# ChenWu98/cycle-diffusion

Measured on AMD Instinct MI355X. Metric: images/sec, SD-v1.4 512px CycleDiffusion 100+100 steps, 1/2/4/8 MI355X, higher is better.
Workload: dtype fp16; 1 GPU; C2: Stable-Diffusion-v1.4-shaped U-Net + KL-f8 VAE, 512x512, custom_steps=99 white_box_steps=100 eta=0.1 skip 0, 1 trial, encoder scale 1, decoder CFG 3; batch_per_gpu=4, global_batch=4, parallelism=dp1, steps_per_launch_set=5, launch_set_cap=16, launch_sets_in_flight_per_gpu=1, images_in_flight_per_gpu=20, distributed=single process, weights=synthetic(seed=0)

## Files before the change

### cycle-diffusion_amd/_ffi.py

```python
import ctypes as C
import os

import numpy as np

_HERE = os.path.dirname(os.path.abspath(__file__))
LIB_PATH = os.path.join(_HERE, "lib", "libcyclediff.so")

CD_NET_UNET_OPENAI, CD_NET_UNET_HO, CD_NET_VAE_KL, CD_NET_CLIP_TEXT, CD_NET_BERT_XTR = 1, 2, 3, 4, 5
CD_NET_OCLIP_TEXT, CD_NET_OCLIP_VISION, CD_NET_INCEPTION_FID, CD_NET_LPIPS = 6, 7, 8, 9
CD_SCHED_DDIM, CD_SCHED_DDPM = 0, 1
CD_PREC_16, CD_PREC_F32, CD_PREC_F32X3 = 0, 1, 2
CD_MASK_QSAMPLE, CD_MASK_ENCODER = 0, 1
MASK_SOURCES = {"q_sample": CD_MASK_QSAMPLE, "encoder": CD_MASK_ENCODER}
ACT_NONE, ACT_SILU, ACT_GELU, ACT_GEGLU, ACT_QGELU, ACT_RELU = 0, 1, 2, 3, 4, 5


class NetDesc(C.Structure):
    _fields_ = [
        ("kind", C.c_int), ("image_size", C.c_int), ("in_channels", C.c_int), ("out_channels", C.c_int),
        ("model_channels", C.c_int), ("num_res_blocks", C.c_int),
        ("n_mult", C.c_int), ("channel_mult", C.c_int * 8),
        ("n_attn", C.c_int), ("attn", C.c_int * 8),
        ("num_heads", C.c_int), ("num_head_channels", C.c_int),
        ("use_spatial_transformer", C.c_int), ("context_dim", C.c_int), ("transformer_depth", C.c_int),
# ... 66 lines not shown
    "cd_net_create": [_VP, C.POINTER(NetDesc), C.POINTER(_I)],
    "cd_net_param_count": [_VP, _I, C.POINTER(_I)],
    "cd_net_param_info": [_VP, _I, _I, C.c_char_p, _I, C.POINTER(_I), C.POINTER(_I64)],
    "cd_net_load_param": [_VP, _I, C.c_char_p, _VP, _I, C.POINTER(_I64)],
    "cd_net_missing_params": [_VP, _I, C.POINTER(_I), C.c_char_p, _I],
    "cd_unet_forward": [_VP, _I, _VP, _VP, _VP, _I, _I, _VP],
    "cd_text_encode": [_VP, _I, _VP, _I, _I, _VP],
    "cd_clip_text_features": [_VP, _I, _VP, _I, _I, _VP],
    "cd_clip_image_features": [_VP, _I, _VP, _I, _VP],
    "cd_inception_features": [_VP, _I, _VP, _I, _I, _VP],
    "cd_lpips": [_VP, _I, _VP, _VP, _I, _I, _I, _VP, _VP],
    "cd_lpips_tap": [_VP, _I, _VP, _I, _I, _I, _I, _VP],
    "cd_vae_encode": [_VP, _I, _VP, _VP, _U64, _I, _I, _I, _F, _VP],
    "cd_vae_decode": [_VP, _I, _VP, _I, _I, _F, _F, _F, _VP],
    "cd_vae_encode_hw": [_VP, _I, _VP, _VP, _U64, _I, _I, _I, _I, _F, _VP],
    "cd_vae_decode_hw": [_VP, _I, _VP, _I, _I, _I, _F, _F, _F, _VP],
    "cd_dpm_encode": [_VP, _I, _I, _VP, _VP, _VP, _I, _F, _I, _I, _VP, _VP, _U64, _I, _VP],
    "cd_ddim_decode": [_VP, _I, _I, _VP, _I, _I, _VP, _VP, _I, _F, _I, _I, _VP, _VP, _U64, _VP],
    "cd_ddim_decode_v": [_VP, _I, _I, _VP, _I, _I, _VP, _VP, _I, _VP, _I, _I, _VP, _VP, _U64, _VP],
    "cd_ddim_invert": [_VP, _I, _I, _VP, _VP, _VP, _I, _F, _I, _I, _VP, _VP, _VP],
    "cd_cycle_translate": [_VP, C.POINTER(TranslateArgs)],
    "cd_ddim_decode_masked": [_VP, _I, _I, _VP, _I, _I, _VP, _VP, _I, _F, _VP, _I, _I, _VP, _VP, _U64, _VP, _VP, _I, _I, _VP, _VP,
                              _U64, _VP],
    "cd_ilvr_decode": [_VP, _I, _I, _VP, _I, _I, _I, _I, _VP, _VP, _U64, _VP, _I, _I, _I, _VP, _VP, _U64, _VP],
    "cd_automask": [_VP, _I, _VP, _VP, _VP, _I, _I, _I, _I, _F, _F, _VP, _U64, _I, _F, _F, _I, _VP, _VP],
    "cd_word_maps": [_VP, _I, _VP, _VP, _I, _I, _VP, _I, _I, _I, _I, _F, _F, _VP, _U64, _I, _I, _I, _VP, C.POINTER(_I)],
    "cd_pix_refine": [_VP, _I, _I, _VP, _I, _I, _VP, _VP, _U64],
    "cd_op_pack_conv_weight": [_VP, _VP, _I, _I, _I, _I, _I, C.POINTER(_VP), C.POINTER(_I), C.POINTER(_I)],
    "cd_op_free": [_VP, _VP],
    "cd_op_conv2d": [_VP, _VP, _I, _VP, _I, _I, _I, _I, _VP, _I, _I, _I, _I, _I, _I, _I, _VP, _VP, _VP, _I, _I, _VP],
    "cd_op_conv2d_16": [_VP, _VP, _I, _VP, _I, _I, _I, _I, _VP, _I, _I, _I, _I, _I, _I, _I, _VP, _VP, _VP, _I, _I, _VP,
                        _VP],
    "cd_op_last_gemm_config": [_VP] + [C.POINTER(_I)] * 5,
    "cd_op_up_phase_reorder": [_VP, _VP, _I, _I, _I, _I, _VP],
    "cd_op_groupnorm": [_VP, _VP, _I, _I, _I, _I, _I, _F, _VP, _VP, _VP, _I, _VP],
    "cd_op_groupnorm_ex": [_VP, _VP, _I, _I, _VP, _I, _I, _I, _I, _I, _F, _VP, _VP, _VP, _I, _I, _VP, _VP, _I, _VP],
    "cd_op_pack_conv_weight_prec": [_VP, _VP, _I, _I, _I, _I, _I, C.POINTER(_VP)],
    "cd_op_conv2d_prec": [_VP, _VP, _I, _I, _VP, _I, _I, _I, _I, _I, _VP, _I, _I, _I, _I, _I, _I, _I, _VP, _VP, _I, _VP, _I, _I,
                          _I, _I, _I, _I, _F, _VP, _VP],
    "cd_op_attention_prec": [_VP, _VP, _VP, _VP, _I, _I, _I, _I, _I, _I, _I, _I, _F, _I, _VP, _I, _I, _VP],
    "cd_op_rows_prec": [_VP, _I, _VP, _I64, _I, _I, _VP, _I, _I, _VP, _VP, _I, _VP],
    "cd_op_resample_prec": [_VP, _I, _VP, _I, _I, _I, _I, _I, _VP],
    "cd_op_layernorm": [_VP, _VP, _I, _I, _VP, _VP, _F, _VP],
    "cd_op_st_entry": [_VP, _VP, _I, _I, _I, _VP, _VP, _F, _VP, _VP, _VP, _VP, _VP, _VP, _VP, _I, _VP, _VP, _VP,
                       C.POINTER(_I)],
    "cd_op_attention": [_VP, _VP, _VP, _VP, _I, _I, _I, _I, _I, _F, _I, _VP],
    "cd_op_cross_attention_ctrl": [_VP, _VP, _VP, _VP, _VP, _VP, _VP, _VP, _VP, _I, _I, _I, _I, _I, _I, _I, _I, _F, _VP],
    "cd_op_cross_attention_ctrl_ex": [_VP, _VP, _VP, _VP, _VP, _VP, _VP, _VP, _VP, _I, _I, _I, _I, _I, _I, _I, _I, _F, _I, _I,
                                      _VP],
    "cd_op_cross_attention_maps": [_VP, _VP, _VP, _VP, _I, _I, _I, _I, _I, _I, _I, _I, _F, _I, _VP],
    "cd_op_attention_ex": [_VP, _VP, _VP, _VP, _I, _I, _I, _I, _I, _I, _I, _I, _I, _I, _F, _I, _VP, _I, _I, _VP],
    "cd_op_lowpass": [_VP, _VP, _I, _I, _I, _I, _VP],
    "cd_op_softmax_rows": [_VP, _VP, _I64, _I, _VP],
    "cd_op_timestep_embedding": [_VP, _VP, _I, _I, _I, _VP],
    "cd_op_sched_step": [_VP, _I, _I, _VP, _VP, _VP, _VP, _I, _F, _VP, _VP, _I, _I, _I, _I, _VP],
    "cd_op_gauss": [_VP, _U64, C.c_uint32, _I64, _I64, _VP],
    "cd_op_automask_reduce": [_VP, _VP, _VP, _I, _I, _I, _I, _I, _F, _F, _I, _VP, _VP, _VP],
    "cd_op_local_blend_mask": [_VP, _VP, _VP, _I, _I, _I, _I, _I, _F, _VP],
    "cd_op_sched_step_masked": [_VP, _I, _VP, _VP, _VP, _I, _F, _VP, _VP, _VP, _I, _I, _F, _F, _VP, _I, _I, _I, _I, _VP, _I],
    "cd_op_sega_guidance": [_VP, _VP, _I, _I, _I, _I, _I, _F, _VP, _VP, _I, _F, _F, _VP, _VP, _VP, _VP, _VP],
    "cd_op_window_gather": [_VP, _VP, _VP, _I, _I, _I, _I, _I, _I, _I, _I, _VP],
    "cd_op_window_fuse": [_VP, _VP, _VP, _I, _I, _I, _I, _I, _I, _I, _I, _VP],
    "cd_op_layout": [_VP, _I, _VP, _VP, _I, _I, _I, _I, _I, _F, _F, _I],
    "cd_op_resample16": [_VP, _I, _VP, _VP, _I, _I, _I, _I],
    "cd_op_copy_rows16": [_VP, _VP, _I, _VP, _I, _I64, _I],
    "cd_op_vec_linear": [_VP, _VP, _I, _VP, _VP, _VP, _I, _I, _I, _I, _I, _I],
# ... 65 lines not shown
```

### cycle-diffusion_amd/csrc/capi_ops.hip

```cpp
#include "capi_internal.h"

namespace {

bf16_t* op_rows16(cd_engine* h, const float* src, int64_t rows, int C) {
  bf16_t* d = (bf16_t*)h->arena.alloc((size_t)rows * C * 2);
  launch_nchw_to_nhwc(h->st, src, d, (int)rows, C, 1, C, 1.f, 0.f, 0);
  return d;
}
Act op_image16(Ctx& c, const float* x, int B, int C, int H, int W, int Cpad) {
  Act a = alloc_act(c, B, H, W, Cpad);
  launch_nchw_to_nhwc(c.st, x, a.p, B, C, H * W, Cpad, 1.f, 0.f, 0);
  return a;
}

bf16_t* op_nan_rows16(cd_engine* h, int64_t rows, int ld) {
  const size_t bytes = (size_t)(rows + 64) * ld * 2;
  bf16_t* t = (bf16_t*)h->arena.alloc(bytes);
  HIP_CHECK(hipMemsetAsync(t, 0xFF, bytes, h->st));
  return t;
}
float* op_nan_buffer(cd_engine* h, size_t n) {
  float* t = (float*)h->arena.alloc(n * sizeof(float));
  launch_fill_f32(h->st, t, __builtin_nanf(""), (int64_t)n);
  return t;
// ... 48 lines not shown
  Act a; a.B = B; a.H = H; a.W = W; a.C = Cpad; a.ld = 2 * Cpad; a.f32 = true; a.split = true;
  a.p = (bf16_t*)h->arena.alloc((size_t)B * H * W * 2 * Cpad * sizeof(bf16_t));
  launch_nchw_to_nhwc_f32(h->st, x, a.pf(), B, C, H * W, Cpad, 1.f, 0.f, 1, h->overflow_dev);
  return a;
}

void op_download_nchw(cd_engine* h, const void* p, bool f32, int ld, float* y, int B, int C, int HW) {
  launch_nhwc_to_nchw(h->st, p, f32 ? 1 : 0, ld, y, B, C, HW, 1.f, 0.f);
}
void op_download(cd_engine* h, const Act& o, size_t floats, void* y) {
  HIP_CHECK(hipMemcpyAsync(y, o.p, floats * 4, hipMemcpyDeviceToDevice, h->st));
  HIP_CHECK(hipStreamSynchronize(h->st));
  h->check_overflow();
}

void conv_out_hw(int H, int W, int KH, int KW, int stride, int pad, bool asym, bool up, int* Ho, int* Wo) {
  const int Hin = up ? 2 * H : H, Win = up ? 2 * W : W;
  *Ho = asym ? (Hin + 1 - KH) / stride + 1 : (Hin + 2 * pad - KH) / stride + 1;
  *Wo = asym ? (Win + 1 - KW) / stride + 1 : (Win + 2 * pad - KW) / stride + 1;
}
Ctx prec_ctx(cd_engine* h, int precision) {
  Ctx c = h->ctx();
  c.f32 = precision != 0; c.x3 = precision == 2;
  return c;
}

void op_conv2d(cd_handle h, const float* x0, int C0, const float* x1, int C1, int B, int H, int W,
               const void* packed_w, int N, int KH, int KW, int stride, int pad, int asym_pad, int up,
               const float* bias, const float* rowvec, const float* resid, int act, int tile, bool out16,
               float* y, float* stats) {
  CD_CHECK(h && x0 && packed_w && y, "bad argument");
  ArenaScope arena_scope(h->arena);
  Ctx c = h->ctx();
  if (up && out16) {
    ConvW* pw = (ConvW*)const_cast<void*>(packed_w);
    h->op_params.add_up_phase(pw);
    h->op_params.refresh_up_phase(h->st, pw);
  }
  ConvW w = *(const ConvW*)packed_w;
  CD_CHECK(w.N == N && w.KH == KH && w.KW == KW, "packed weight does not match the call");
  w.b = const_cast<float*>(bias);
  Act a0 = op_image16(c, x0, B, C0, H, W, x1 ? C0 : round_up(C0, 32));
  Act a1;
  if (x1) a1 = op_image16(c, x1, B, C1, H, W, C1);
  ConvOpts o; o.stride = stride; o.pad = pad; o.asym = asym_pad != 0; o.up = up != 0; o.tile = tile;
  if (act & 0x400) {
    CD_CHECK(out16 && conv_ln_fold_available(c, w, (int64_t)B * H * W) , "LayerNorm fold needs tile 30 shapes");
    o.ln_fold = true;
    act &= ~0x400;
  }
  o.act = act;
  o.out_f32 = !out16;
  o.want_stats = stats != nullptr;
  int Ho, Wo;
  conv_out_hw(H, W, KH, KW, stride, pad, asym_pad != 0, up != 0, &Ho, &Wo);
  const int Nout = w.geglu ? N / 2 : N;
  if (rowvec) { o.rowvec = rowvec; o.rowvec_ld = N; o.rows_per_vec = Ho * Wo; }
  Act r;
  if (resid) {
    r = op_image16(c, resid, B, Nout, Ho, Wo, Nout);
    o.resid = &r;
  }
  Act out = conv_fwd(c, w, a0, x1 ? &a1 : nullptr, o);
  op_download_nchw(h, out.p, !out16, out.ld, y, B, Nout, Ho * Wo);
  if (stats) {
    CD_CHECK(out.stats, "this convolution produces no GroupNorm statistics (GEGLU, or rows %% 32 != 0)");
    HIP_CHECK(hipMemcpyAsync(stats, out.stats, (size_t)(out.rows() / 32) * 2 * Nout * sizeof(float),
                             hipMemcpyDeviceToDevice, h->st));
  }
}

void op_cross_attention_ctrl(cd_engine* h, const float* q_own, const float* q_src, const float* k_own,
                             const float* k_src, const float* v_own, const float* mapper, const float* alpha,
                             const float* weight, int B, int B_src, int B_ctrl, int H, int Tq, int L, int L_buf, int D,
                             float scale, int q_log2, int opad, float* o) {
  CD_CHECK(h && q_own && q_src && k_own && k_src && v_own && mapper && alpha && weight && o, "bad argument");
  CD_CHECK(B > 0 && B_src > 0 && B_ctrl > 0 && H > 0 && Tq > 0 && D > 0 && L > 0 && L_buf >= L, "bad argument");
  CD_CHECK(opad >= 0 && opad % 4 == 0, "opad: a multiple of 4 elements");
  ArenaScope arena_scope(h->arena);
  const int C = H * D, ldo = C + opad;
  CtrlAttnParams p;
  p.q_own = op_rows16(h, q_own, (int64_t)B * Tq, C); p.q_src = op_rows16(h, q_src, (int64_t)B_src * Tq, C);
  p.k_own = op_rows16(h, k_own, (int64_t)B * L_buf, C); p.k_src = op_rows16(h, k_src, (int64_t)B_src * L_buf, C);
  const bf16_t* vb16 = op_rows16(h, v_own, (int64_t)B * L, C);
  bf16_t* va = (bf16_t*)h->arena.alloc((size_t)B * L * C * 2);
  bf16_t* vb = (bf16_t*)h->arena.alloc((size_t)B * L * C * 2);
  launch_ctrl_values(h->st, vb16, mapper, alpha, weight, B, B_ctrl, L, C, va, vb);
  bf16_t* ob = op_nan_rows16(h, (int64_t)B * Tq, ldo);
  p.va = va; p.vb = vb; p.o = ob;
  p.B = B; p.B_src = B_src; p.H = H; p.Tq = Tq; p.L = L; p.D = D;
  p.ldq = C; p.ldk = C; p.ldv = C; p.ldo = ldo;
  p.q_bs = (int64_t)Tq * C; p.k_bs = (int64_t)L_buf * C; p.v_bs = (int64_t)L * C; p.o_bs = (int64_t)Tq * ldo;
  p.scale = scale; p.q_log2 = q_log2 != 0;
  launch_cross_attention_ctrl(h->st, p);
  op_download_nchw(h, ob, false, ldo, o, B * Tq, ldo, 1);
// ... 35 lines not shown
int cd_op_conv2d_16(cd_handle h, const float* x0, int C0, const float* x1, int C1, int B, int H, int W,
                    const void* packed_w, int N, int KH, int KW, int stride, int pad, int asym_pad, int up,
                    const float* bias, const float* rowvec, const float* resid, int act, int tile, float* y,
                    float* stats) {
  CD_API_BEGIN
  enter_engine(h);
  op_conv2d(h, x0, C0, x1, C1, B, H, W, packed_w, N, KH, KW, stride, pad, asym_pad, up, bias, rowvec, resid, act, tile,
            true, y, stats);
  CD_API_END
}

int cd_op_up_phase_reorder(cd_handle h, const float* x, int B, int C, int H, int W, float* y) {
  CD_API_BEGIN
  enter_engine(h);
  CD_CHECK(h && x && y && B > 0 && H > 0 && W > 0 && C > 0 && C % 8 == 0, "bad argument");
  ArenaScope arena_scope(h->arena);
  Ctx c = h->ctx();
  Act a = op_image16(c, x, 4 * B, C, H, W, C);
  Act o = alloc_act(c, B, 2 * H, 2 * W, C);
  launch_up_phase_reorder(h->st, a.p, o.p, B, H, W, C, o.ld);
  op_download_nchw(h, o.p, false, o.ld, y, B, C, 4 * H * W);
  CD_API_END
}

int cd_op_last_gemm_config(cd_handle h, int* tile_id, int* bk, int* splitk, int* chm, int* tile_group) {
  CD_API_BEGIN
  CD_CHECK(h, "bad argument");
  const GemmLaunchInfo li = conv_gemm_last_launch();
  if (tile_id) *tile_id = li.tile_id;
  if (bk) *bk = li.bk;
  if (splitk) *splitk = li.splitk;
  if (chm) *chm = li.chm;
  if (tile_group) *tile_group = li.tile_group;
  CD_API_END
}

int cd_op_groupnorm(cd_handle h, const float* x, int B, int C, int H, int W, int G, float eps,
                    const float* gamma, const float* beta, const float* film, int silu, float* y) {
  CD_API_BEGIN
  enter_engine(h);
  CD_CHECK(h && x && y && G == 32, "bad argument (G must be 32)");
  ArenaScope arena_scope(h->arena);
  Ctx c = h->ctx();
  Act a = op_image16(c, x, B, C, H, W, C);
  GNW w; w.g = const_cast<float*>(gamma); w.b = const_cast<float*>(beta); w.C = C; w.eps = eps;
  Act o = groupnorm_fwd(c, w, a, nullptr, silu != 0, film, film ? 2 * C : 0);
  op_download_nchw(h, o.p, false, o.ld, y, B, C, H * W);
  CD_API_END
}

int cd_op_groupnorm_ex(cd_handle h, const float* x0, int C0, int pad0, const float* x1, int C1, int pad1, int B, int H,
                       int W, float eps, const float* gamma, const float* beta, const float* film, int film_ld, int silu,
                       const float* stats0, const float* stats1, int precision, void* y) {
  CD_API_BEGIN
  enter_engine(h);
  CD_CHECK(h && x0 && gamma && beta && y && B > 0 && H > 0 && W > 0 && C0 > 0 && pad0 >= 0 && pad1 >= 0, "bad argument");
  CD_CHECK(x1 ? C1 > 0 : (C1 == 0 && !stats1), "bad argument (second source)");
  CD_CHECK(precision >= 0 && precision <= 2 && film_ld >= 0, "bad argument (precision 0 = 16-bit, 1 = fp32, 2 = fp32 split)");
  const int align = precision ? 4 : 8;
  CD_CHECK((C0 + pad0) % align == 0 && (C1 + pad1) % align == 0, "row strides must be multiples of %d elements", align);
  ArenaScope arena_scope(h->arena);
  Ctx c = prec_ctx(h, precision);
  const int HW = H * W, C = C0 + C1;
  Act a0 = c.f32 ? op_upload_nhwc(h, x0, B, C0, C0, C0 + pad0, H, W) : op_upload_nhwc16(h, x0, B, C0, C0 + pad0, H, W);
  a0.stats = const_cast<float*>(stats0);
  Act a1;
// ... 942 lines not shown
```

### cycle-diffusion_amd/csrc/conv_gemm.hip

```cpp
#include <stdio.h>
#include <stdlib.h>
#include <string.h>

#include <algorithm>
#include <map>
#include <mutex>
#include <string>

#include "common.h"
#include "kernels.h"

namespace cd {

namespace gemm_detail {

typedef const __attribute__((address_space(1))) void* gptr_t;
typedef __attribute__((address_space(3))) void* lptr_t;

template <int BM, int BN, int BK, int WM, int WN, int NSTAGE>
struct TileCfg {
  static constexpr int NW = WM * WN;
  static constexpr int CPR = BK / 8;
  static constexpr int RPI = 64 / CPR;
  static constexpr int A_IPW = BM / RPI / NW;
  static constexpr int B_IPW = BN / RPI / NW;
  static constexpr int LPT = A_IPW + B_IPW;
  static constexpr int TM = BM / WM, TN = BN / WN;
  static constexpr int MT = TM / 32, NT = TN / 32;
  static constexpr int KS = BK / 16;
  static constexpr int SWZ_SHIFT = (CPR == 8) ? 1 : 2;
  static constexpr int CW = TN >= 64 ? 64 : TN;
  static constexpr int EPI_LD = CW + 4;
  static constexpr int PF = (MT * NT >= 8) ? 1 : 2;
  static constexpr int A_BYTES = BM * BK * 2, B_BYTES = BN * BK * 2;
  static constexpr int STAGE_BYTES = A_BYTES + B_BYTES;
  static constexpr int EPI_BYTES = NW * TM * EPI_LD * 4;
  static constexpr int LDS_BYTES = STAGE_BYTES * NSTAGE > EPI_BYTES ? STAGE_BYTES * NSTAGE : EPI_BYTES;
  static constexpr int TAB_BIAS_I = (BN / 4 + 63) / 64;
  static constexpr int TAB_RV_I = ((BM / 32) * (BN / 4) + 63) / 64;
  static constexpr bool HAS_TAB = LDS_BYTES + (TAB_BIAS_I + TAB_RV_I) * 1024 <= 160 * 1024;
  static constexpr int TAB_BYTES = HAS_TAB ? (TAB_BIAS_I + TAB_RV_I) * 1024 : 0;
  static_assert(NW == 4 || NW == 8 || NW == 16, "4, 8 or 16 waves");
  static_assert(A_IPW >= 1 && B_IPW >= 1, "tile too small for the wave count");
  static_assert(A_IPW * RPI * NW == BM && B_IPW * RPI * NW == BN, "tile rows must split evenly over waves");
  static_assert(MT >= 1 && NT >= 1, "wave tile");
  static_assert(NSTAGE >= 2 && NSTAGE <= 8, "ring depth");
  static_assert((NSTAGE - 2) * LPT <= 63, "vmcnt field");
  static_assert(LDS_BYTES + TAB_BYTES <= 160 * 1024, "LDS");
};

template <int N>
__device__ __forceinline__ void wait_vmcnt_barrier() {
  asm volatile("s_waitcnt vmcnt(%0)\n\ts_barrier" ::"n"(N) : "memory");
}

__device__ __forceinline__ __amdgpu_buffer_rsrc_t uniform_rsrc(const void* base, int bytes) {
  const uint64_t u = (uint64_t)base;
  const uint32_t lo = (uint32_t)__builtin_amdgcn_readfirstlane((int)(uint32_t)u);
  const uint32_t hi = (uint32_t)__builtin_amdgcn_readfirstlane((int)(uint32_t)(u >> 32));
  return __builtin_amdgcn_make_buffer_rsrc((void*)(((uint64_t)hi << 32) | lo), 0, __builtin_amdgcn_readfirstlane(bytes), 0x00020000);
}

__device__ __forceinline__ bool fast_epilogue(const ConvGemmParams& p) {
  return p.act == ACT_NONE && !p.out_f32 && !p.resid_f32 && (p.N & 7) == 0 && (p.out_ld & 7) == 0 &&
         (((uintptr_t)p.out | (uintptr_t)p.resid | (uintptr_t)p.rowvec) & 15) == 0 && (p.o_bs & 7) == 0 &&
         (!p.resid || (p.resid_ld & 7) == 0) &&
         (!p.rowvec || ((p.rowvec_ld & 3) == 0 && (p.rows_per_vec >= p.M || (p.rows_per_vec & 31) == 0)));
}

template <int BM, int BN, int BK, int WM, int WN, int NSTAGE, bool CHM = false>
__global__ __launch_bounds__(64 * WM * WN, (WM * WN == 4 && BK == 32 && NSTAGE == 3 && BM * BN >= 128 * 256) ? 2 : 1) void k_conv_gemm(ConvGemmParams p) {
#if defined(__HIP_DEVICE_COMPILE__)
  using T = TileCfg<BM, BN, BK, WM, WN, NSTAGE>;
  constexpr int CPR = T::CPR, RPI = T::RPI, A_IPW = T::A_IPW, B_IPW = T::B_IPW, NW = T::NW;
  constexpr int MT = T::MT, NT = T::NT, KS = T::KS, TM = T::TM, TN = T::TN, LPT = T::LPT;
  extern __shared__ __attribute__((aligned(16))) char smem[];

  const int tid = threadIdx.x;
  const int lane = tid & 63;
  const int wave = __builtin_amdgcn_readfirstlane(tid >> 6);
  const int wm = wave / WN, wn = wave % WN;

  const int tiles_n = (p.N + BN - 1) / BN;
  const int tiles_m = (p.M + BM - 1) / BM;
  const int ntiles = tiles_m * tiles_n;
  int tile;
  {
    const int bid = blockIdx.x;
    const int q = ntiles >> 3, r = ntiles & 7;
    const int xcd = bid & 7, loc = bid >> 3;
    tile = (xcd < r ? xcd * (q + 1) : r * (q + 1) + (xcd - r) * q) + loc;
  }
  const bool nmajor = (int64_t)p.N * p.Ktot > (int64_t)p.B * p.Hs * p.Ws * (p.C0 + p.C1);
  int tm, tn;
  if (p.tile_group > 0) {
    const int width = p.tile_group * tiles_n;
    const int grp = tile / width, within = tile - grp * width;
    const int first_m = grp * p.tile_group;
    const int gsz = (tiles_m - first_m) < p.tile_group ? (tiles_m - first_m) : p.tile_group;
    tn = within / gsz; tm = first_m + (within - tn * gsz);
  } else if (nmajor) { tn = tile / tiles_m; tm = tile - tn * tiles_m; }
  else { tm = tile / tiles_n; tn = tile - tm * tiles_n; }
  const int m0 = tm * BM, n0 = tn * BN;
// ... 212 lines not shown
  wait_vmcnt_barrier<(NSTAGE - 1) * LPT + TABI>();

  bf16x8 af[KS][MT], bfr[KS][NT];
  auto read_frags = [&](int slot, int ks) {
    const char* Ab = As + slot * T::A_BYTES;
    const char* Bb = Bs + slot * T::B_BYTES;
#pragma unroll
    for (int i = 0; i < MT; ++i) {
      const int row = wm * TM + i * 32 + frow;
      const int ch = (ks * 2 + fhalf) ^ ((row >> T::SWZ_SHIFT) & (CPR - 1));
      af[ks][i] = *(const bf16x8*)(Ab + row * (BK * 2) + ch * 16);
    }
#pragma unroll
    for (int j = 0; j < NT; ++j) {
      const int row = wn * TN + j * 32 + frow;
      const int ch = (ks * 2 + fhalf) ^ ((row >> T::SWZ_SHIFT) & (CPR - 1));
      bfr[ks][j] = *(const bf16x8*)(Bb + row * (BK * 2) + ch * 16);
    }
  };
#pragma unroll
  for (int q = 0; q < PF; ++q) read_frags(0, q);
  __builtin_amdgcn_sched_barrier(0);

  int cur = 0;
  int fill = 0;
  for (int kt = kt0; kt < kt1; ++kt) {
    const int nslot = (cur + 1 == NSTAGE) ? 0 : cur + 1;
#pragma unroll
    for (int ks = 0; ks < KS; ++ks) {
      const int jrel = (ks - SYNC + KS) % KS;
      auto mfma_range = [&](int lo, int hi) __attribute__((always_inline)) {
#pragma unroll
        for (int n = 0; n < NMF; ++n)
          if (n >= lo && n < hi) acc[n / NT][n % NT] = CD_MFMA_32x32x16(af[ks][n / NT], bfr[ks][n % NT], acc[n / NT][n % NT]);
      };
      if (ks == SYNC) {
        mfma_range(0, HALF);
        asm volatile("s_waitcnt vmcnt(%0) lgkmcnt(0)\n\ts_barrier" ::"n"((NSTAGE - 2) * LPT) : "memory");
        prepare(kt + NSTAGE);
        fill = cur;
#pragma unroll
        for (int l = 0; l < LPT / SPREAD; ++l) issue(l, fill);
        mfma_range(HALF, NMF);
      } else {
        if (SPREAD > 1 && (ks > SYNC || kt != kt0)) {
#pragma unroll
          for (int l = (jrel * LPT) / SPREAD; l < ((jrel + 1) * LPT) / SPREAD; ++l) issue(l, fill);
        }
        mfma_range(0, NMF);
      }
      if (ks + PF < KS) read_frags(cur, ks + PF);
      else read_frags(nslot, ks + PF - KS);
      __builtin_amdgcn_sched_barrier(0);
    }
    cur = nslot;
  }
  asm volatile("s_waitcnt vmcnt(0)" ::: "memory");
  __syncthreads();

  if (nsplit > 1) {
    constexpr int TILE_BYTES = BM * BN * 4;
    constexpr int kSc1 = 16;
    typedef __attribute__((ext_vector_type(4))) unsigned int u32x4;
    float* part0 = p.sk_scratch + ((int64_t)zb * ntiles + tile) * nsplit * (BM * BN);
    const __amdgpu_buffer_rsrc_t rsp = __builtin_amdgcn_make_buffer_rsrc((void*)part0, 0, kRange, 0x00020000);
#pragma unroll
    for (int i = 0; i < MT; ++i)
#pragma unroll
      for (int j = 0; j < NT; ++j)
#pragma unroll
        for (int q = 0; q < 4; ++q) {
          const f32x4 v = {acc[i][j][4 * q], acc[i][j][4 * q + 1], acc[i][j][4 * q + 2], acc[i][j][4 * q + 3]};
          const int off = sidx * TILE_BYTES + (((i * NT + j) * 4 + q) * (64 * NW) + tid) * 16;
          __builtin_amdgcn_raw_buffer_store_b128(__builtin_bit_cast(u32x4, v), rsp, off, 0, kSc1);
        }
    asm volatile("s_waitcnt vmcnt(0)" ::: "memory");
    __syncthreads();
    int* flag = p.sk_flags + zb * ntiles + tile;
    if (tid == 0) *(volatile int*)smem = __hip_atomic_fetch_add(flag, 1, __ATOMIC_RELAXED, __HIP_MEMORY_SCOPE_AGENT);
    __syncthreads();
    const int arrived = *(volatile int*)smem;
    __syncthreads();
    if (arrived != nsplit - 1) return;
    if (tid == 0) __hip_atomic_store(flag, 0, __ATOMIC_RELAXED, __HIP_MEMORY_SCOPE_AGENT);
#pragma unroll
    for (int i = 0; i < MT; ++i)
#pragma unroll
      for (int j = 0; j < NT; ++j)
#pragma unroll
        for (int r = 0; r < 16; ++r) acc[i][j][r] = 0.0f;
// ... 346 lines not shown
        }
        if (p.stats) {
#pragma unroll
          for (int e = 0; e < 8; ++e) { ssum[e] += v[e]; ssq[e] += v[e] * v[e]; }
        }
        }
        if (p.stats && ((r0 + rpp) & 31) == 0) {
          for (int o = vpr; o < 64; o <<= 1) {
#pragma unroll
            for (int e = 0; e < 8; ++e) { ssum[e] += __shfl_xor(ssum[e], o); ssq[e] += __shfl_xor(ssq[e], o); }
          }
          const int rb = (m0 + wm * TM + r0 + rpp - 32) >> 5;
          if (vr == 0 && n < p.N && (rb << 5) < p.M) {
            float* sp = p.stats + ((int64_t)zb * ((p.M + 31) >> 5) + rb) * 2 * p.N + n;
#pragma unroll
            for (int e = 0; e < 8; ++e) if (e < nvalid) { sp[e] = ssum[e]; sp[p.N + e] = ssq[e]; }
          }
#pragma unroll
          for (int e = 0; e < 8; ++e) { ssum[e] = 0.f; ssq[e] = 0.f; }
        }
      }
    }
  }
#endif
}


inline bool takes_channel_major(const ConvGemmParams& p) {
  const int64_t a_bytes = (int64_t)p.B * p.Hs * p.Ws * (p.C0 + p.C1) * 2;
  return p.korder != 0 && p.KH * p.KW > 1 && p.KH <= 8 && p.KW <= 8 && !p.up && !p.up_phase &&
         (p.korder == 2 || (p.Hs * p.Ws >= 4096 && a_bytes >= (32ll << 20)));
}

template <int BM, int BN, int BK, int WM, int WN, int NSTAGE>
int launch_cfg(hipStream_t st, const ConvGemmParams& p) {
  using T = TileCfg<BM, BN, BK, WM, WN, NSTAGE>;
  const int tiles = ceil_div(p.M, BM) * ceil_div(p.N, BN);
  const int split = p.splitk > 1 ? p.splitk : 1;
  constexpr int kLds = T::LDS_BYTES + T::TAB_BYTES;
  const bool chm = takes_channel_major(p);
  static PerDeviceOnce attr_once;
  auto kern0 = k_conv_gemm<BM, BN, BK, WM, WN, NSTAGE, false>;
  auto kern1 = k_conv_gemm<BM, BN, BK, WM, WN, NSTAGE, true>;
  attr_once([&]() {
    HIP_CHECK(hipFuncSetAttribute((const void*)kern0, hipFuncAttributeMaxDynamicSharedMemorySize, kLds));
    HIP_CHECK(hipFuncSetAttribute((const void*)kern1, hipFuncAttributeMaxDynamicSharedMemorySize, kLds));
  });
  auto kern = chm ? kern1 : kern0;
  if (split > 1) {
    const SplitKWorkspace& ws = g_conv_splitk;
    CD_CHECK(p.sk_scratch && p.sk_flags, "conv_gemm: split-K without workspace");
    CD_CHECK((size_t)tiles * p.nbatch * split * BM * BN * 4 <= ws.scratch_bytes && tiles * p.nbatch <= ws.nflags,
             "conv_gemm: split-K workspace too small");
  }
  hipLaunchKernelGGL(kern, dim3(tiles, split, p.nbatch), dim3(64 * T::NW), kLds, st, p);
  return 0;
}

struct CfgInfo { int id, BM, BN, TN; const char* name; };
const CfgInfo kCfgs[] = {
    {1, 128, 128, 64, "128x128 w2x2 s2"},
    {2, 128, 64, 64, "128x64 w4x1 s2"},
    {3, 64, 64, 32, "64x64 w2x2 s2"},
    {4, 128, 128, 64, "128x128 w2x2 s3"},
    {5, 256, 128, 64, "256x128 w4x2 s3"},
    {6, 128, 256, 64, "128x256 w2x4 s3"},
    {7, 128, 64, 64, "128x64 w4x1 s4"},
    {8, 64, 64, 32, "64x64 w2x2 s4"},
    {9, 256, 64, 64, "256x64 w8x1 s4"},
    {10, 128, 128, 64, "128x128 w2x2 s4"},
    {11, 64, 128, 64, "64x128 w2x2 s4"},
    {12, 128, 64, 64, "128x64 w4x1 s3"},
    {13, 256, 64, 64, "256x64 w8x1 s3"},
    {14, 128, 128, 64, "128x128 w4x2 s3"},
    {15, 64, 64, 32, "64x64 w2x2 s8"},
    {16, 128, 64, 64, "128x64 w4x1 s6"},
    {17, 64, 128, 64, "64x128 w2x2 s6"},
    {18, 256, 128, 32, "256x128 w4x4 s3"},
    {19, 256, 128, 64, "256x128 w8x2 s3"},
    {20, 256, 320, 160, "256x320 w4x2 s2"},
    {21, 128, 320, 160, "128x320 w2x2 s2"},
// ... 66 lines not shown
thread_local const char* g_last_cfg = "";
thread_local GemmLaunchInfo g_last_launch;

int device_cu_count() {
  static std::atomic<int> ncu_of[64];
  int dev = 0;
  if (hipGetDevice(&dev) != hipSuccess) return 256;
  int n = ncu_of[dev & 63].load(std::memory_order_relaxed);
  if (!n) {
    hipDeviceProp_t prop;
    n = (hipGetDeviceProperties(&prop, dev) == hipSuccess && prop.multiProcessorCount > 0) ? prop.multiProcessorCount : 256;
    ncu_of[dev & 63].store(n, std::memory_order_relaxed);
  }
  return n;
}

int pick_config(const ConvGemmParams& p) {
  const int64_t ncu = device_cu_count();
  const int64_t t128 = (int64_t)ceil_div(p.M, 128) * ceil_div(p.N, 128) * p.nbatch;
  const int64_t t12864 = (int64_t)ceil_div(p.M, 128) * ceil_div(p.N, 64) * p.nbatch;
  if (p.act == ACT_GEGLU) return (2 * t128 >= 3 * ncu) ? 1 : 2;
  if (2 * t128 >= 3 * ncu && p.N % 128 == 0) return 1;
  if (t128 >= 2 * ncu) return 1;
  if (t12864 >= ncu) return 2;
  return 3;
}

}
using namespace gemm_detail;

const char* conv_gemm_last_config() { return g_last_cfg; }
GemmLaunchInfo conv_gemm_last_launch() { return g_last_launch; }

thread_local KernelProfiler* g_conv_prof = nullptr;

void KernelProfiler::next_pair(hipEvent_t* a, hipEvent_t* b, double fl, const std::string& what) {
  labels.push_back(what);
  if (used + 2 > (int)events.size()) {
    const size_t old = events.size();
    events.resize(old + 1024);
    for (size_t i = old; i < events.size(); ++i) HIP_CHECK(hipEventCreate(&events[i]));
  }
  *a = events[used]; *b = events[used + 1];
  used += 2;
  flops.push_back(fl);
}
void KernelProfiler::collect(int* launches, double* total_ms, double* total_flops) {
  double ms = 0, fl = 0;
  for (int i = 0; i + 1 < used; i += 2) {
    HIP_CHECK(hipEventSynchronize(events[i + 1]));
    float t = 0;
    HIP_CHECK(hipEventElapsedTime(&t, events[i], events[i + 1]));
    ms += t; fl += flops[i / 2];
    if (verbose) {
      auto& e = per_shape[labels[i / 2]];
      e.n += 1; e.ms += t; e.flops += flops[i / 2];
    }
  }
  if (verbose) {
    std::vector<std::pair<std::string, Entry>> v(per_shape.begin(), per_shape.end());
    std::sort(v.begin(), v.end(), [](const auto& x, const auto& y) { return x.second.ms > y.second.ms; });
    fprintf(stderr, "[conv_gemm] %d launches %.3f ms %.1f TFLOP/s\n", used / 2, ms, fl / ms * 1e-9);
    for (auto& kv : v)
      fprintf(stderr, "  %-58s n=%4d %8.3f ms %7.1f us/launch %7.1f TF/s\n", kv.first.c_str(), kv.second.n,
              kv.second.ms, kv.second.ms / kv.second.n * 1e3, kv.second.flops / kv.second.ms * 1e-9);
    per_shape.clear();
// ... 276 lines not shown
```

### cycle-diffusion_amd/csrc/kernels.h

```cpp
#pragma once
#include <map>
#include <string>
#include <vector>

#include "common.h"

namespace cd {

struct StepCoef {
  float sa, s1a, sap, dirc, sigma, r, t_mask;
  int t;
};
enum { SCHED_DDIM = 0, SCHED_DDPM = 1 };

struct EpsHat {
  const float* p = nullptr;
  int64_t sb = 0, sc = 0, sp = 0;
  int cfg = 0;
  float g = 1.f;
  const float* gvec = nullptr;
};

struct StepGeom {
  int B = 0, C = 0, HW = 0;
// ... 199 lines not shown
  int act = ACT_NONE;
  void* out = nullptr;
  int out_ld = 0;
  int out_f32 = 0;
  float* stats = nullptr;
  const bf16_t* zeros = nullptr;
  int ln_fold = 0;
  float ln_eps = 1e-5f;
  int tile = 0;
  float prof_flop_scale = 1.f;
  int splitk = 0;
  float* sk_scratch = nullptr;
  int* sk_flags = nullptr;
  int korder = 1;
  int tile_group = 0;
  int up_phase = 0;
  int w_ps = 0;
};
struct SplitKWorkspace {
  float* scratch = nullptr;
  size_t scratch_bytes = 0;
  int* flags = nullptr;
  int nflags = 0;
};
extern thread_local SplitKWorkspace g_conv_splitk;
void launch_conv_gemm(hipStream_t st, const ConvGemmParams& p);
const char* conv_gemm_last_config();
struct GemmLaunchInfo {
  int tile_id = 0;
  int bk = 0;
  int splitk = 1;
  int chm = 0;
  int tile_group = 0;
};
GemmLaunchInfo conv_gemm_last_launch();
void launch_up_phase_weights(hipStream_t st, const bf16_t* w, bf16_t* out, int Npad, int Cpad);
int conv_gemm_num_configs();
const char* conv_gemm_config_name(int id);

struct LinStreamParams {
  const bf16_t* a = nullptr; int lda = 0;
  const bf16_t* wfrag = nullptr;
  const float* bias = nullptr;
  const bf16_t* resid = nullptr; int ldr = 0;
  bf16_t* out = nullptr; int ldo = 0;
  float* stats = nullptr;
  int M = 0, N = 0;
  float ln_eps = 1e-5f;
  int nsplit = 0, hw = 0;
  bf16_t* vt = nullptr; int vt_ld = 0;
  int64_t vt_bytes = 0;
  const float* gn_coef = nullptr;
};
constexpr int kLinStreamTile = 30;
bool lin_stream_supports(const ConvGemmParams& p);
void launch_lin_stream(hipStream_t st, const ConvGemmParams& p);
bool lin_stream_entry_supports(int64_t M, int hw, int lda);
void launch_lin_stream_qkv(hipStream_t st, const bf16_t* a, int lda, int M, int hw, const bf16_t* wfrag, const float* bias,
                           bf16_t* qk, bf16_t* vt, int vt_ld, bool ln_fold, float ln_eps);
void launch_lin_stream_gn(hipStream_t st, const bf16_t* a, int lda, int M, int hw, const float* gn_coef, const bf16_t* wfrag,
                          const float* bias, bf16_t* out, int ldo);
void launch_fold_ln(hipStream_t st, const bf16_t* w, int ldw, const float* gamma, const float* beta, const float* bias,
                    bf16_t* w_out, float* bias_out, int N, int Kc);
void launch_pack_wfrag(hipStream_t st, const bf16_t* w, int ldw, bf16_t* out, int N);

struct KernelProfiler {
  bool enabled = false;
  std::vector<hipEvent_t> events;
// ... 169 lines not shown
```

### include/cyclediff.h

```cpp
#ifndef CYCLEDIFF_H
#define CYCLEDIFF_H
#include <stddef.h>
#include <stdint.h>

#ifdef __cplusplus
extern "C" {
#endif

typedef struct cd_engine* cd_handle;

enum { CD_NET_UNET_OPENAI = 1, CD_NET_UNET_HO = 2, CD_NET_VAE_KL = 3, CD_NET_CLIP_TEXT = 4, CD_NET_BERT_XTR = 5,
       CD_NET_OCLIP_TEXT = 6, CD_NET_OCLIP_VISION = 7, CD_NET_INCEPTION_FID = 8, CD_NET_LPIPS = 9 };
enum { CD_SCHED_DDIM = 0, CD_SCHED_DDPM = 1 };
enum { CD_PREC_16 = 0, CD_PREC_F32 = 1, CD_PREC_F32X3 = 2 };
enum { CD_MASK_QSAMPLE = 0, CD_MASK_ENCODER = 1 };

typedef struct cd_net_desc {
  int kind;
  int image_size;
  int in_channels, out_channels;
  int model_channels;
  int num_res_blocks;
  int n_mult;  int channel_mult[8];
  int n_attn;  int attn[8];
// ... 156 lines not shown
  int n_win;
  const int32_t* win_host;
} cd_translate_args;

int cd_cycle_translate(cd_handle h, const cd_translate_args* a);

int cd_ilvr_decode(cd_handle h, int net, int sched_kind, const float* z, int z_slots, int n_eps, int B, int K,
                   const cd_step_coef* coef_host, const float* noise_tail, uint64_t seed, const float* ref, int B_ref,
                   int down_n, int range_t, const float* qsample_coef_host, const float* ref_noise, uint64_t ref_seed,
                   float* x_out);

int cd_automask(cd_handle h, int net, const float* x0, const float* ctx_src, const float* ctx_tgt, int ctx_len, int B,
                int n_draws, int t, float qa, float qb, const float* noise, uint64_t seed, int max_rows, float ratio, float thr,
                int dilate, float* map_out, float* keep_out);

int cd_word_maps(cd_handle h, int net, const float* x0, const float* ctx, int ctx_len, int B, const float* sel, int B_sel,
                 int N, int n_draws, int t, float qa, float qb, const float* noise, uint64_t seed, int max_rows,
                 int min_side, int max_side, float* maps_out , int* n_layers_out);

int cd_pix_refine(cd_handle h, int net, int sched_kind, float* x, int B, int R,
                  const cd_step_coef* coef_host, const float* noise, uint64_t seed);

int cd_op_pack_conv_weight(cd_handle h, const float* w_host, int N, int Cin, int KH, int KW, int geglu,
                           void** packed_dev, int* Npad, int* Cpad);
int cd_op_free(cd_handle h, void* dev);
int cd_op_conv2d(cd_handle h, const float* x0, int C0, const float* x1, int C1, int B, int H, int W,
                 const void* packed_w, int N, int KH, int KW, int stride, int pad, int asym_pad, int up,
                 const float* bias, const float* rowvec, const float* resid, int act, int tile, float* y);
int cd_op_conv2d_16(cd_handle h, const float* x0, int C0, const float* x1, int C1, int B, int H, int W,
                    const void* packed_w, int N, int KH, int KW, int stride, int pad, int asym_pad, int up,
                    const float* bias, const float* rowvec, const float* resid, int act, int tile, float* y,
                    float* stats);
int cd_op_last_gemm_config(cd_handle h, int* tile_id, int* bk, int* splitk, int* chm, int* tile_group);
int cd_op_up_phase_reorder(cd_handle h, const float* x, int B, int C, int H, int W, float* y);
int cd_op_groupnorm(cd_handle h, const float* x, int B, int C, int H, int W, int G, float eps,
                    const float* gamma, const float* beta, const float* film, int silu, float* y);
int cd_op_groupnorm_ex(cd_handle h, const float* x0, int C0, int pad0, const float* x1, int C1, int pad1, int B, int H,
                       int W, float eps, const float* gamma, const float* beta, const float* film, int film_ld, int silu,
                       const float* stats0, const float* stats1, int precision, void* y);
int cd_op_pack_conv_weight_prec(cd_handle h, const float* w_host, int N, int Cin, int KH, int KW, int geglu,
                                void** packed_dev);
int cd_op_conv2d_prec(cd_handle h, const float* x0, int C0, int pad0, const float* x1, int C1, int pad1, int B, int H, int W,
                      const void* packed_w, int N, int KH, int KW, int stride, int pad, int asym_pad, int up,
                      const float* bias, const float* rowvec, int rowvec_shared, const float* resid, int resid_pad, int act,
                      int raw_geglu, int tile, int precision, int via_split_rows, float alpha, float* y, float* stats);
int cd_op_attention_prec(cd_handle h, const float* q, const float* k, const float* v, int B, int H, int Tq, int Tk, int D,
                         int padq, int padk, int padv, float scale, int q_log2, const float* obias, int mode, int precision,
                         void* o);
int cd_op_rows_prec(cd_handle h, int op, const float* x0, int64_t rows, int C0, int pad0, const float* x1, int C1, int pad1,
                    const float* gamma, const float* beta, int precision, void* y);
int cd_op_resample_prec(cd_handle h, int op, const float* x, int B, int C, int H, int W, int precision, void* y);
int cd_op_layernorm(cd_handle h, const float* x, int rows, int C, const float* gamma, const float* beta,
                    float eps, float* y);
int cd_op_st_entry(cd_handle h, const float* x, int B, int H, int W, const float* gn_gamma, const float* gn_beta,
                   float gn_eps, const void* w_in, const float* b_in, const float* ln_gamma, const float* ln_beta,
                   const void* w_qk, const void* w_v, const float* v_bias, int stages, float* h_out, float* qk_out,
                   float* vt_out, int* stages_run);
int cd_op_attention(cd_handle h, const float* q, const float* k, const float* v, int B, int H, int Tq,
                    int Tk, int D, float scale, int use_transpose_kernel, float* o);
int cd_op_cross_attention_ctrl(cd_handle h, const float* q_own, const float* q_src, const float* k_own, const float* k_src,
                               const float* v_own, const float* mapper, const float* alpha, const float* weight, int B,
                               int B_src, int B_ctrl, int H, int Tq, int L, int L_buf, int D, float scale, float* o);
int cd_op_cross_attention_ctrl_ex(cd_handle h, const float* q_own, const float* q_src, const float* k_own, const float* k_src,
                                  const float* v_own, const float* mapper, const float* alpha, const float* weight, int B,
                                  int B_src, int B_ctrl, int H, int Tq, int L, int L_buf, int D, float scale, int q_log2,
                                  int opad, float* o);
// ... 64 lines not shown
```

Before: 3.591 images/s.

## Add direct-to-global GEGLU epilogue for 256x256x64 conv GEMM tile

Adds a kernel variant for the 256x256 BK64 tile in which the MFMA operands are swapped, so each lane holds rows of output. It then applies the bias from the LDS table and the GEGLU gating in registers, and writes packed bf16 rows straight to global memory with buffer stores and a permlane32 swap. This skips the final __syncthreads and the LDS-staged epilogue for GEGLU feed-forward GEMMs without residual, stats or split-K. The path is on by default, can be switched off through an env var or API call, and adds test hooks for padded output rows. The risk is uncoalesced or partial stores and extra register pressure in the new template instance.

Result: no change. 3.609 images/s, median of 6 (+0.5%).

```diff
diff --git a/cycle-diffusion_amd/_ffi.py b/cycle-diffusion_amd/_ffi.py
--- a/cycle-diffusion_amd/_ffi.py
+++ b/cycle-diffusion_amd/_ffi.py
@@ -122,6 +122,8 @@
     "cd_op_conv2d_16": [_VP, _VP, _I, _VP, _I, _I, _I, _I, _VP, _I, _I, _I, _I, _I, _I, _I, _VP, _VP, _VP, _I, _I, _VP,
                         _VP],
     "cd_op_last_gemm_config": [_VP] + [C.POINTER(_I)] * 5,
+    "cd_op_set_direct_epilogue": [_VP, _I],
+    "cd_op_last_gemm_epilogue": [_VP, C.POINTER(_I)],
     "cd_op_up_phase_reorder": [_VP, _VP, _I, _I, _I, _I, _VP],
     "cd_op_groupnorm": [_VP, _VP, _I, _I, _I, _I, _I, _F, _VP, _VP, _VP, _I, _VP],
     "cd_op_groupnorm_ex": [_VP, _VP, _I, _I, _VP, _I, _I, _I, _I, _I, _F, _VP, _VP, _VP, _I, _I, _VP, _VP, _I, _VP],
diff --git a/cycle-diffusion_amd/csrc/capi_ops.hip b/cycle-diffusion_amd/csrc/capi_ops.hip
--- a/cycle-diffusion_amd/csrc/capi_ops.hip
+++ b/cycle-diffusion_amd/csrc/capi_ops.hip
@@ -104,6 +104,9 @@
   CD_CHECK(h && x0 && packed_w && y, "bad argument");
   ArenaScope arena_scope(h->arena);
   Ctx c = h->ctx();
+  const int out_pad = (tile & (1 << 20)) ? 64 : 0;
+  tile &= (1 << 20) - 1;
+  CD_CHECK(!out_pad || (out16 && !stats), "padded output rows: 16-bit output without statistics");
   if (up && out16) {
     ConvW* pw = (ConvW*)const_cast<void*>(packed_w);
     h->op_params.add_up_phase(pw);
@@ -133,6 +136,7 @@
     r = op_image16(c, resid, B, Nout, Ho, Wo, Nout);
     o.resid = &r;
   }
+  if (out_pad) { o.out = op_nan_rows16(h, (int64_t)B * Ho * Wo, Nout + out_pad); o.out_ld = Nout + out_pad; }
   Act out = conv_fwd(c, w, a0, x1 ? &a1 : nullptr, o);
   op_download_nchw(h, out.p, !out16, out.ld, y, B, Nout, Ho * Wo);
   if (stats) {
@@ -234,6 +238,20 @@
   if (splitk) *splitk = li.splitk;
   if (chm) *chm = li.chm;
   if (tile_group) *tile_group = li.tile_group;
+  CD_API_END
+}
+
+int cd_op_set_direct_epilogue(cd_handle h, int mask) {
+  CD_API_BEGIN
+  CD_CHECK(h, "bad argument");
+  conv_gemm_set_direct_epilogue(mask);
+  CD_API_END
+}
+
+int cd_op_last_gemm_epilogue(cd_handle h, int* direct) {
+  CD_API_BEGIN
+  CD_CHECK(h, "bad argument");
+  if (direct) *direct = conv_gemm_last_launch().direct;
   CD_API_END
 }
 
diff --git a/cycle-diffusion_amd/csrc/conv_gemm.hip b/cycle-diffusion_amd/csrc/conv_gemm.hip
--- a/cycle-diffusion_amd/csrc/conv_gemm.hip
+++ b/cycle-diffusion_amd/csrc/conv_gemm.hip
@@ -16,6 +16,8 @@
 
 typedef const __attribute__((address_space(1))) void* gptr_t;
 typedef __attribute__((address_space(3))) void* lptr_t;
+
+constexpr int kDirectEpiDefault = DIRECT_EPI_ALL;
 
 template <int BM, int BN, int BK, int WM, int WN, int NSTAGE>
 struct TileCfg {
@@ -68,7 +70,12 @@
          (!p.rowvec || ((p.rowvec_ld & 3) == 0 && (p.rows_per_vec >= p.M || (p.rows_per_vec & 31) == 0)));
 }
 
-template <int BM, int BN, int BK, int WM, int WN, int NSTAGE, bool CHM = false>
+inline int direct_epilogue_class(const ConvGemmParams& p, int nt, bool has_tab) {
+  if (!has_tab || p.act != ACT_GEGLU || p.out_f32 || p.resid || p.stats || p.rowvec || p.splitk > 1) return 0;
+  return ((nt & 1) == 0 && (p.N & 63) == 0 && (p.out_ld & 7) == 0 && (((uintptr_t)p.out) & 15) == 0 && (p.o_bs & 7) == 0) ? DIRECT_EPI_GEGLU : 0;
+}
+
+template <int BM, int BN, int BK, int WM, int WN, int NSTAGE, bool CHM = false, bool DIR = false>
 __global__ __launch_bounds__(64 * WM * WN, (WM * WN == 4 && BK == 32 && NSTAGE == 3 && BM * BN >= 128 * 256) ? 2 : 1) void k_conv_gemm(ConvGemmParams p) {
 #if defined(__HIP_DEVICE_COMPILE__)
   using T = TileCfg<BM, BN, BK, WM, WN, NSTAGE>;
@@ -347,7 +354,10 @@
       auto mfma_range = [&](int lo, int hi) __attribute__((always_inline)) {
 #pragma unroll
         for (int n = 0; n < NMF; ++n)
-          if (n >= lo && n < hi) acc[n / NT][n % NT] = CD_MFMA_32x32x16(af[ks][n / NT], bfr[ks][n % NT], acc[n / NT][n % NT]);
+          if (n >= lo && n < hi) {
+            if constexpr (DIR) acc[n / NT][n % NT] = CD_MFMA_32x32x16(bfr[ks][n % NT], af[ks][n / NT], acc[n / NT][n % NT]);
+            else acc[n / NT][n % NT] = CD_MFMA_32x32x16(af[ks][n / NT], bfr[ks][n % NT], acc[n / NT][n % NT]);
+          }
       };
       if (ks == SYNC) {
         mfma_range(0, HALF);
@@ -371,6 +381,56 @@
     cur = nslot;
   }
   asm volatile("s_waitcnt vmcnt(0)" ::: "memory");
+  if constexpr (DIR) {
+    static_assert(T::HAS_TAB && (NT & 1) == 0, "bias from the tile's LDS table; a value / gate pair of blocks per wave");
+    static_assert(BN * 4 <= T::TAB_BIAS_I * 1024 && T::TAB_BIAS_I * 1024 <= T::TAB_BYTES, "every bias index lies inside the table");
+    typedef __attribute__((ext_vector_type(4))) unsigned int u32x4d;
+    int lane_d = lane;
+    asm volatile("" : "+v"(lane_d));
+    const int drow = lane_d & 31, dhalf = lane_d >> 5;
+    if (p.alpha != 1.0f) {
+#pragma unroll
+      for (int i = 0; i < MT; ++i)
+#pragma unroll
+        for (int j = 0; j < NT; ++j)
+#pragma unroll
+          for (int r = 0; r < 16; ++r) acc[i][j][r] *= p.alpha;
+    }
+    char* outp = (char*)p.out + (int64_t)zb * p.o_bs * 2;
+    const int mw = m0 + wm * TM;
+    int rows_ok = p.M - mw;
+    rows_ok = rows_ok < 0 ? 0 : (rows_ok > TM ? TM : rows_ok);
+    const int nw = n0 + wn * TN;
+    const int ocol0 = nw >> 1;
+    const int ocols = (p.N - nw) >> 1;
+    const float* TB = (const float*)(smem + T::LDS_BYTES) + wn * TN + 4 * dhalf;
+    const __amdgpu_buffer_rsrc_t rs_o = uniform_rsrc(outp + (int64_t)mw * p.out_ld * 2, rows_ok * p.out_ld * 2);
+    const unsigned vo_row = (unsigned)((drow * p.out_ld + ocol0) * 2);
+#pragma unroll
+    for (int i = 0; i < MT; ++i)
+#pragma unroll
+      for (int j = 0; j < NT; j += 2)
+#pragma unroll
+        for (int qp = 0; qp < 2; ++qp) {
+          const float* tb = TB + j * 32 + 16 * qp;
+          const f32x4 bv0 = *(const f32x4*)tb, bv1 = *(const f32x4*)(tb + 8);
+          const f32x4 bg0 = *(const f32x4*)(tb + 32), bg1 = *(const f32x4*)(tb + 40);
+          float va[8], ga[8], v[8];
+#pragma unroll
+          for (int e = 0; e < 4; ++e) {
+            va[e] = acc[i][j][8 * qp + e] + bv0[e]; va[4 + e] = acc[i][j][8 * qp + 4 + e] + bv1[e];
+            ga[e] = acc[i][j + 1][8 * qp + e] + bg0[e]; ga[4 + e] = acc[i][j + 1][8 * qp + 4 + e] + bg1[e];
+          }
+          mul_gelu8(va, ga, v);
+          const uint4 pk = pack8(v);
+          const auto s0 = __builtin_amdgcn_permlane32_swap(pk.x, pk.z, false, false);
+          const auto s1 = __builtin_amdgcn_permlane32_swap(pk.y, pk.w, false, false);
+          const int c = (j / 2) * 32 + 16 * qp + 8 * dhalf;
+          __builtin_amdgcn_raw_buffer_store_b128((u32x4d){s0[0], s1[0], s0[1], s1[1]}, rs_o,
+                                                 c < ocols ? vo_row + (unsigned)((i * 32 * p.out_ld + c) * 2) : kInvalid, 0, 0);
+        }
+    return;
+  }
   __syncthreads();
 
   if (nsplit > 1) {
@@ -783,6 +843,13 @@
          (p.korder == 2 || (p.Hs * p.Ws >= 4096 && a_bytes >= (32ll << 20)));
 }
 
+extern thread_local GemmLaunchInfo g_last_launch;
+
+template <int BM, int BN, int BK, int WM, int WN, int NSTAGE>
+constexpr bool has_direct_epilogue() {
+  return BM == 256 && BN == 256 && BK == 64 && WM == 4 && WN == 2 && NSTAGE == 2;
+}
+
 template <int BM, int BN, int BK, int WM, int WN, int NSTAGE>
 int launch_cfg(hipStream_t st, const ConvGemmParams& p) {
   using T = TileCfg<BM, BN, BK, WM, WN, NSTAGE>;
@@ -798,6 +865,15 @@
     HIP_CHECK(hipFuncSetAttribute((const void*)kern1, hipFuncAttributeMaxDynamicSharedMemorySize, kLds));
   });
   auto kern = chm ? kern1 : kern0;
+  int direct = 0;
+  if constexpr (has_direct_epilogue<BM, BN, BK, WM, WN, NSTAGE>()) {
+    auto kernd = k_conv_gemm<BM, BN, BK, WM, WN, NSTAGE, false, true>;
+    static PerDeviceOnce attr_once_d;
+    attr_once_d([&]() { HIP_CHECK(hipFuncSetAttribute((const void*)kernd, hipFuncAttributeMaxDynamicSharedMemorySize, kLds)); });
+    if (!chm) direct = direct_epilogue_class(p, T::NT, T::HAS_TAB) & conv_gemm_direct_epilogue_mask();
+    if (direct) kern = kernd;
+  }
+  g_last_launch.direct = direct;
   if (split > 1) {
     const SplitKWorkspace& ws = g_conv_splitk;
     CD_CHECK(p.sk_scratch && p.sk_flags, "conv_gemm: split-K without workspace");
@@ -930,6 +1006,15 @@
 const char* conv_gemm_last_config() { return g_last_cfg; }
 GemmLaunchInfo conv_gemm_last_launch() { return g_last_launch; }
 
+static std::atomic<int> g_direct_epi_override{-1};
+int conv_gemm_direct_epilogue_mask() {
+  const int o = g_direct_epi_override.load(std::memory_order_relaxed);
+  if (o >= 0) return o & DIRECT_EPI_ALL;
+  static const int env = [] { const char* e = getenv("CYCLEDIFF_DIRECT_EPI"); return (e && e[0] ? atoi(e) : kDirectEpiDefault) & DIRECT_EPI_ALL; }();
+  return env;
+}
+void conv_gemm_set_direct_epilogue(int mask) { g_direct_epi_override.store(mask < 0 ? -1 : mask, std::memory_order_relaxed); }
+
 thread_local KernelProfiler* g_conv_prof = nullptr;
 
 void KernelProfiler::next_pair(hipEvent_t* a, hipEvent_t* b, double fl, const std::string& what) {
diff --git a/cycle-diffusion_amd/csrc/kernels.h b/cycle-diffusion_amd/csrc/kernels.h
--- a/cycle-diffusion_amd/csrc/kernels.h
+++ b/cycle-diffusion_amd/csrc/kernels.h
@@ -255,8 +255,12 @@
   int splitk = 1;
   int chm = 0;
   int tile_group = 0;
+  int direct = 0;
 };
 GemmLaunchInfo conv_gemm_last_launch();
+enum { DIRECT_EPI_GEGLU = 1, DIRECT_EPI_ALL = 1 };
+int conv_gemm_direct_epilogue_mask();
+void conv_gemm_set_direct_epilogue(int mask);
 void launch_up_phase_weights(hipStream_t st, const bf16_t* w, bf16_t* out, int Npad, int Cpad);
 int conv_gemm_num_configs();
 const char* conv_gemm_config_name(int id);
diff --git a/include/cyclediff.h b/include/cyclediff.h
--- a/include/cyclediff.h
+++ b/include/cyclediff.h
@@ -212,6 +212,8 @@
                     const float* bias, const float* rowvec, const float* resid, int act, int tile, float* y,
                     float* stats);
 int cd_op_last_gemm_config(cd_handle h, int* tile_id, int* bk, int* splitk, int* chm, int* tile_group);
+int cd_op_set_direct_epilogue(cd_handle h, int mask);
+int cd_op_last_gemm_epilogue(cd_handle h, int* direct);
 int cd_op_up_phase_reorder(cd_handle h, const float* x, int B, int C, int H, int W, float* y);
 int cd_op_groupnorm(cd_handle h, const float* x, int B, int C, int H, int W, int G, float eps,
                     const float* gamma, const float* beta, const float* film, int silu, float* y);
```
